# Lcrypto/mod-interleaveavx_multithreads-FAID

Measured on AMD Instinct MI355X. Metric: decoded Gb/s @ 10 iters, 50G-PON LDPC; FER match vs AVX512 ref, higher is better.
Workload: dtype i8

## Files before the change

### include/lnsfaid.h

```cpp
#ifndef LNSFAID_H
#define LNSFAID_H

#include <stddef.h>
#include <stdint.h>

#ifdef __cplusplus
extern "C" {
#endif

#define LNSFAID_GROUP 32

#define LNSFAID_OK 0
#define LNSFAID_E_INVAL (-1)
#define LNSFAID_E_CODE (-2)
#define LNSFAID_E_NOMEM (-3)
#define LNSFAID_E_HIP (-4)
#define LNSFAID_E_NODEVICE (-5)
#define LNSFAID_E_INTERNAL (-6)

typedef struct lnsfaid_code {
    int32_t n_var;
    int32_t n_check;
    int32_t n_edges;
    int32_t z;
// ... 162 lines not shown
int lnsfaid_io_buffers(lnsfaid_ctx* ctx, int8_t** d_fixInput, int8_t** d_decodedBits, lnsfaid_group_stats** d_stats);

int lnsfaid_host_register(void* ptr, size_t bytes);
int lnsfaid_host_unregister(void* ptr);

int lnsfaid_read_stats(lnsfaid_ctx* ctx, lnsfaid_group_stats* stats, size_t n_groups);

#define LNSFAID_COMM_ID_BYTES 128
int lnsfaid_comm_unique_id(uint8_t id[LNSFAID_COMM_ID_BYTES]);
int lnsfaid_comm_init(lnsfaid_ctx* ctx, int32_t n_ranks, int32_t rank, const uint8_t id[LNSFAID_COMM_ID_BYTES]);
int lnsfaid_comm_attach(lnsfaid_ctx* ctx, void* nccl_comm);
int lnsfaid_comm_destroy(lnsfaid_ctx* ctx);
int lnsfaid_allreduce_counters(lnsfaid_ctx* ctx, uint64_t counters[4]);

int lnsfaid_select_kernel(lnsfaid_ctx* ctx, int32_t rows_per_lane);
int lnsfaid_kernel_rows_per_lane(const lnsfaid_ctx* ctx);

int lnsfaid_select_waves(lnsfaid_ctx* ctx, int32_t waves_per_codeword);
int lnsfaid_kernel_waves(const lnsfaid_ctx* ctx);

#define LNSFAID_MSG_REGISTERS 1
#define LNSFAID_MSG_HBM 2
int lnsfaid_select_message_store(lnsfaid_ctx* ctx, int32_t where);
int lnsfaid_message_store(const lnsfaid_ctx* ctx);

#define LNSFAID_ZERO_SHIFT_ON 1
#define LNSFAID_ZERO_SHIFT_OFF 2
#define LNSFAID_ZERO_SHIFT_LOOP 3
#define LNSFAID_ZERO_SHIFT_STATIC 4
int lnsfaid_select_zero_shift(lnsfaid_ctx* ctx, int32_t mode);
int lnsfaid_zero_shift_groups(const lnsfaid_ctx* ctx, int32_t* groups, int32_t n);
int lnsfaid_code_zero_shift_order(const lnsfaid_code* code, int32_t* groups, int32_t* order);

int lnsfaid_kernel_residency(lnsfaid_ctx* ctx, int32_t* workgroups_per_cu, int32_t* lds_limit);


int lnsfaid_kernel_time(lnsfaid_ctx* ctx, double* out_ms, uint64_t* out_launches, int32_t reset);

void* lnsfaid_stream(lnsfaid_ctx* ctx);

const char* lnsfaid_strerror(int err);
const char* lnsfaid_last_hip_error(void);
const char* lnsfaid_version(void);

#ifdef __cplusplus
}
#endif
#endif
```

### mod-interleaveavx_multithreads-faid_amd/csrc/lnsfaid_capi.hip

```cpp
#include <hip/hip_runtime.h>

#include <dlfcn.h>
#include <rccl/rccl.h>

#include <cstdio>
#include <cstdlib>
#include <cstring>
#include <new>
#include <vector>

#include "lnsfaid_device.h"
#include "lnsfaid_quantise.h"
#include "lnsfaid_swar.h"

extern "C" hipError_t lf_launch_decode(int method, int uniform_w, const LfKernelArgs* args, size_t lds_bytes,
                                       hipStream_t stream);
extern "C" const void* lf_decode_func(int method, int uniform_w);
extern "C" int lf_decode_threads(void);
extern "C" const void* lf_decode4_func(int method, int ef, int rm);
extern "C" int lf_decode4_threads(void);
extern "C" hipError_t lf_launch_decode4(int method, int ef, int rm, const LfKernelArgs* args, size_t lds_bytes, hipStream_t stream);
extern "C" int lf_decode4_rm_layers(void);
extern "C" const void* lf_decode4cw_func(int method, int ef, int rm);
extern "C" hipError_t lf_launch_decode4cw(int method, int ef, int rm, const LfCwArgs* args, size_t lds_bytes, hipStream_t stream);
// ... 127 lines not shown
    int fe_interleave = 1;
    int fe_exact = 0;
    int fe_prefec = 0;
    unsigned long long* d_fe_prefec_frames = nullptr;
    unsigned long long* d_fe_prefec_acc = nullptr;
    uint2* d_cap_cnt = nullptr;
    unsigned long long* d_cap_meta = nullptr;
    unsigned long long* h_cap_meta = nullptr;
    size_t cap_slots = 0;
    uint32_t* d_cap_slots = nullptr;
    lnsfaid_error_record* d_cap_records = nullptr;
    int8_t* d_cap_payload = nullptr;
    unsigned long long* d_fec_acc = nullptr;
    unsigned long long* h_fec_acc = nullptr;
    int enc_state = 0;
    uint32_t* d_enc_sup = nullptr;
    uint32_t* d_enc_off = nullptr;
    unsigned long long* d_fe_keys = nullptr;
};

static int stream_wait(lnsfaid_ctx* ctx)
{
    if (sync_blocking()) {
        HIP_TRY(hipEventRecord(ctx->ev_block, ctx->stream));
        HIP_TRY(hipEventSynchronize(ctx->ev_block));
    } else {
        HIP_TRY(hipStreamSynchronize(ctx->stream));
    }
    return LNSFAID_OK;
}

static int weight_class(int w) { return w == 3 ? 0 : (w == 6 ? 1 : (w == 11 ? 2 : 3)); }

static int build_code(const lnsfaid_code* code, LfDevCode* out)
{
    memset(out, 0, sizeof(*out));
    if (!code || !code->pos_vn || !code->deg || !code->deg_rows) return LNSFAID_E_INVAL;
    const int Z = code->z, N = code->n_var, M = code->n_check, E = code->n_edges;
    if (Z != LF_Z) return LNSFAID_E_CODE;
    if (N <= 0 || M <= 0 || N % Z || M % Z || M >= N) return LNSFAID_E_CODE;
    const int nbr = M / Z, nbc = N / Z, K = N - M;
    if (nbr > LF_MAX_BR || nbc > LF_MAX_BC) return LNSFAID_E_CODE;
    if (K % 4 || M % 4 || N % LF_T) return LNSFAID_E_CODE;
    if (code->puncture_tail < 0 || code->puncture_tail > N) return LNSFAID_E_CODE;
    std::vector<int> row_deg;
    row_deg.reserve(M);
    long e_total = 0;
    for (int k = 0; k < code->nb_degres; ++k) {
        if (code->deg_rows[k] < 0 || code->deg[k] < 2 || code->deg[k] > LF_MAX_DEG) return LNSFAID_E_CODE;
        for (int i = 0; i < code->deg_rows[k]; ++i) { row_deg.push_back(code->deg[k]); e_total += code->deg[k]; }
    }
    if ((int)row_deg.size() != M || e_total != E) return LNSFAID_E_CODE;

    size_t e = 0;
    for (int br = 0; br < nbr; ++br) {
        const int deg = row_deg[(size_t)br * Z];
        out->deg[br] = deg;
        const uint16_t* row0 = code->pos_vn + e;
        for (int j = 0; j < 64; ++j) out->sbtab[br][j] = 0u;
        for (int j = 0; j < 32; ++j) out->sbplain[br][j] = 0u;
        int prev_cb = -1;
        for (int j = 0; j < deg; ++j) {
            const int cb = row0[j] / Z, sh = row0[j] % Z;
            if (row0[j] >= N || cb <= prev_cb) return LNSFAID_E_CODE;
            prev_cb = cb;
            out->circ[br][j].sb = (uint32_t)cb * (uint32_t)Z + (uint32_t)sh;
// ... 3 lines not shown
            out->cbtab[br][j] = (uint32_t)cb * (uint32_t)Z;
            if (out->col_weight[cb] >= LF_MAX_COLW) return LNSFAID_E_CODE;
            out->colcirc[cb][out->col_weight[cb]++] = (uint32_t)br | ((uint32_t)sh << 8);
        }
        for (int i = 0; i < Z; ++i) {
            if (row_deg[(size_t)br * Z + i] != deg) return LNSFAID_E_CODE;
            for (int j = 0; j < deg; ++j) {
                const uint32_t sb = out->circ[br][j].sb;
                const int want = (int)(sb / (uint32_t)Z * (uint32_t)Z + (sb % (uint32_t)Z + (uint32_t)i) % (uint32_t)Z);
                if (code->pos_vn[e + (size_t)i * deg + j] != want) return LNSFAID_E_CODE;
            }
        }
        e += (size_t)deg * Z;
        for (int j = 0; j < 32; ++j) out->zsbplain[br][j] = 0u;
        int n = 0;
        for (int zero = 1; zero >= 0; --zero)
            for (int j = 0; j < deg; ++j)
                if ((out->s4tab[br][j] == 0u) == (zero != 0)) {
                    out->zsbplain[br][n] = out->sbplain[br][j];
                    out->zs4tab[br][n] = out->s4tab[br][j];
                    out->zcbtab[br][n] = out->cbtab[br][j];
                    ++n;
                }
        int n_zero = 0;
        while (n_zero < deg && out->zs4tab[br][n_zero] == 0u) ++n_zero;
        out->zinst[br] = lf_decode4z_inst(deg, n_zero / 4);
    }
    {
        const int nw = N / 32, pw = M / 32;
        const uint32_t hard0 = lf_lds_off_hard(N), zero = lf_lds_off_zero(N, nw, pw);
        if (lf_lds_bytes(N, nw, pw) > 0xffffu) return LNSFAID_E_CODE;
        for (int br = 0; br < LF_MAX_BR; ++br)
            for (int j = 0; j < LF_MAX_DEG; ++j)
                for (int k = 0; k < 8; ++k) {
                    uint2 e; e.x = zero | (zero << 16); e.y = 0;
                    if (br < nbr && j < out->deg[br]) {
                        const uint32_t sb = out->circ[br][j].sb, cb = sb / (uint32_t)Z, sh = sb % (uint32_t)Z;
                        const uint32_t o = (32u * (uint32_t)k + sh) & 255u, q = o >> 5;
                        e.x = (hard0 + 4u * (cb * 8u + q)) | ((hard0 + 4u * (cb * 8u + ((q + 1u) & 7u))) << 16);
                        e.y = o & 31u;
                    }
                    out->synw[br][j][k] = e;
                }
    }
    for (int br = 0; br < nbr; ++br)
        for (int j = 0; j < out->deg[br]; ++j)
            out->circ[br][j].wclass = (uint32_t)weight_class(out->col_weight[out->circ[br][j].sb / (uint32_t)Z]);
    out->n_var = N; out->n_check = M; out->k_info = K; out->nbr = nbr; out->nbc = nbc;
    out->puncture_tail = code->puncture_tail;
    out->n_words = N / 32; out->p_words = M / 32;
    return LNSFAID_OK;
}

static void build_wcols(LfDevCode* code, int W)
{
    code->n_wcols = 0;
    for (int cb = 0; cb < code->nbc; ++cb)
        if (code->col_weight[cb] == W) code->wcol[code->n_wcols++] = cb;
    bool seen[LF_MAX_BC] = {};
    for (int br = 0; br < LF_MAX_BR; ++br) {
        code->era_edges[br] = 0;
        for (int j = 0; br < code->nbr && j < code->deg[br]; ++j) {
            const int cb = (int)(code->circ[br][j].sb / LF_Z);
            if (code->col_weight[cb] == W && !seen[cb]) { seen[cb] = true; code->era_edges[br] |= 1u << j; }
        }
    }
}

static int build_cfg(const lnsfaid_cfg* cfg, LfDevCfg* out)
{
    if (!cfg) return LNSFAID_E_INVAL;
    if (cfg->decode_method < 0 || cfg->decode_method > 5) return LNSFAID_E_INVAL;
    if (cfg->max_iteration < 0 || cfg->max_iteration > (1 << 20)) return LNSFAID_E_INVAL;
    if (cfg->max_bf_iter < 0 || cfg->max_bf_iter > (1 << 20)) return LNSFAID_E_INVAL;
    if (cfg->regular_col_weight < 0 || cfg->regular_col_weight > LF_MAX_COLW) return LNSFAID_E_INVAL;
    memset(out, 0, sizeof(*out));
    out->method = cfg->decode_method;
    out->max_iter = cfg->max_iteration;
    out->factor_1 = cfg->decode_method == 0 ? (int16_t)cfg->factor_1 : (int8_t)cfg->factor_1;
    out->factor_2 = cfg->decode_method == 0 ? (int16_t)cfg->factor_2 : (int8_t)cfg->factor_2;
    out->floor_err_count = cfg->floor_err_count;
    out->floor_iter_thresh = cfg->floor_iter_thresh;
    out->ef = cfg->ef_elimination;
    out->max_bf = (cfg->decode_method == 0 || cfg->decode_method == 1) ? 0 : cfg->max_bf_iter;
    out->L0 = cfg->bf_L0; out->L1 = cfg->bf_L1; out->alpha = cfg->bf_alpha; out->delta = cfg->bf_delta;
    out->W = cfg->regular_col_weight;
    out->hard2_thr = cfg->hard2_threshold;
    out->vote_cap = (int8_t)cfg->bf_vote_cap;
    if ((cfg->decode_method == 1 || cfg->decode_method == 3 || cfg->decode_method == 4)
        && ((int8_t)cfg->factor_1 < 0 || (int8_t)cfg->factor_2 < 1)) return LNSFAID_E_INVAL;
    if (cfg->decode_method == 5 && cfg->ef_elimination != 1) return LNSFAID_E_INVAL;
    if (cfg->decode_method == 2 && (cfg->ef_elimination < 0 || cfg->ef_elimination > 2)) return LNSFAID_E_INVAL;
    if (cfg->decode_method != 2 && cfg->decode_method != 5 && cfg->ef_elimination != 0) return LNSFAID_E_INVAL;
    out->uniform_w = 1;
    for (int it = 0; it < 6; ++it)
        for (int w = 0; w < 4; ++w) {
            for (int a = 0; a < 8; ++a) {
                const int v = cfg->v2c_map[it][w][a], ve = cfg->v2c_map_ef[it][w][a];
// ... 257 lines not shown
    ctx->zero_shift = mode;
    return LNSFAID_OK;
}

extern "C" int lnsfaid_zero_shift_groups(const lnsfaid_ctx* ctx, int32_t* groups, int32_t n)
{
    if (!ctx || n < 0 || (n > 0 && !groups)) return LNSFAID_E_INVAL;
    const bool on = use_zero_shift(ctx);
    for (int br = 0; br < n; ++br) groups[br] = (on && br < ctx->hcode.nbr) ? layer_zero_groups(ctx, br) : 0;
    return on ? (use_static_layers(ctx) ? 2 : 1) : 0;
}

extern "C" int lnsfaid_code_zero_shift_order(const lnsfaid_code* code, int32_t* groups, int32_t* order)
{
    LfDevCode* dc = new (std::nothrow) LfDevCode;
    if (!dc) return LNSFAID_E_NOMEM;
    const int rc = build_code(code, dc);
    if (rc) { delete dc; return rc; }
    const int nbr = dc->nbr;
    for (int br = 0; br < nbr; ++br) {
        int n_zero = 0;
        while (n_zero < dc->deg[br] && dc->zs4tab[br][n_zero] == 0u) ++n_zero;
        if (groups) groups[br] = n_zero / 4;
        for (int j = 0; order && j < LF_MAX_DEG; ++j) {
            order[br * LF_MAX_DEG + j] = -1;
            for (int i = 0; j < dc->deg[br] && i < dc->deg[br]; ++i)
                if (dc->cbtab[br][i] == dc->zcbtab[br][j] && dc->s4tab[br][i] == dc->zs4tab[br][j]) order[br * LF_MAX_DEG + j] = i;
        }
    }
    delete dc;
    return nbr;
}

static bool cw_possible(const lnsfaid_ctx* ctx) { return ctx->waves_per_cw != 2 && use_kernel4(ctx); }

static bool packed_kernel(const lnsfaid_ctx* ctx) { return use_kernel4(ctx) && !use_kernel5(ctx); }

static const void* selected_kernel(const lnsfaid_ctx* ctx, int* threads, int rule, bool packed = false)
{
    if (packed) {
        *threads = lf_decode4_threads();
        return lf_decode4p_func(ctx->hcfg.method, ctx->hcfg.ef, use_msg_registers(ctx) ? 1 : 0, rule == LNSFAID_STOP_CODEWORD ? 1 : 0);
    }
    if (rule == LNSFAID_STOP_CODEWORD) {
        *threads = lf_decode4_threads();
        return cw_possible(ctx) ? lf_decode4cw_func(ctx->hcfg.method, ctx->hcfg.ef, use_msg_registers(ctx) ? 1 : 0) : nullptr;
    }
    if (use_kernel5(ctx)) {
        *threads = lf_decode5_threads();
        return lf_decode5_func(ctx->hcfg.method);
    }
    if (use_zero_shift(ctx)) {
        *threads = lf_decode4_threads();
        return use_static_layers(ctx) ? lf_decode4s_func(ctx->hcfg.method) : lf_decode4z_func(ctx->hcfg.method);
    }
    if (use_kernel4(ctx)) {
        *threads = lf_decode4_threads();
        return lf_decode4_func(ctx->hcfg.method, ctx->hcfg.ef, use_msg_registers(ctx) ? 1 : 0);
    }
    *threads = lf_decode_threads();
    return lf_decode_func(ctx->hcfg.method, ctx->hcfg.uniform_w);
}

extern "C" int lnsfaid_select_message_store(lnsfaid_ctx* ctx, int32_t where)
{
    if (!ctx || where < 0 || where > LNSFAID_MSG_HBM) return LNSFAID_E_INVAL;
// ... 1562 lines not shown
```

### mod-interleaveavx_multithreads-faid_amd/csrc/lnsfaid_device.h

```cpp
#ifndef LNSFAID_DEVICE_H
#define LNSFAID_DEVICE_H

#include <stdint.h>

#include "lnsfaid.h"

#define LF_Z 256
#define LF_T 128
#define LF_MAX_BR 32
#define LF_MAX_DEG 24
#define LF_MAX_BC 256
#define LF_MAX_COLW 16

#define LF_DONE 0x40000000
#define LF_PROG_MASK 0x0fffffff

#define LF_JCODE_A(j) ((j) < 16 ? (j) : (j) + 16)
#define LF_JCODE_B(j) ((j) < 16 ? (j) + 16 : (j) + 32)

struct LfCirc {
    uint32_t sb;
    uint32_t wclass;
};

struct LfDevCode {
    int32_t n_var, n_check, k_info, nbr, nbc, puncture_tail, n_words , p_words ;
    int32_t n_wcols;
    int32_t deg[LF_MAX_BR];
    LfCirc circ[LF_MAX_BR][LF_MAX_DEG];
    uint32_t sbtab[LF_MAX_BR][64];
    uint32_t sbplain[LF_MAX_BR][32];
    uint32_t s4tab[LF_MAX_BR][LF_MAX_DEG];
    uint32_t cbtab[LF_MAX_BR][LF_MAX_DEG];
    uint2 synw[LF_MAX_BR][LF_MAX_DEG][8];
    int32_t col_weight[LF_MAX_BC];
    int32_t wcol[LF_MAX_BC];
    uint32_t era_edges[LF_MAX_BR];
    uint32_t colcirc[LF_MAX_BC][LF_MAX_COLW];
    uint32_t zsbplain[LF_MAX_BR][32];
    uint32_t zs4tab[LF_MAX_BR][LF_MAX_DEG];
    uint32_t zcbtab[LF_MAX_BR][LF_MAX_DEG];
    int32_t zinst[LF_MAX_BR];
};

struct LfDevCfg {
    int32_t method, max_iter, factor_1, factor_2, floor_err_count, floor_iter_thresh, ef, max_bf;
    int32_t L0, L1, alpha, delta, W, hard2_thr, vote_cap;
    int32_t uniform_w;
    int32_t bf_fast;
    int32_t nms_fits;
    uint32_t nms_t[4];
    uint32_t lut_lo[6][4], lut_hi[6][4];
    uint32_t lut_ef_lo[6][4], lut_ef_hi[6][4];
};

struct LfLaneState {
    int32_t Th, l0, l1, t;
};

struct LfKernelArgs {
    const LfDevCode* code;
    const LfDevCfg* cfg;
    const int8_t* fix_input;
    int8_t* decoded;
    int8_t* st_en;
    uint4* st_rows;
    uint32_t* st_bits;
    LfLaneState* st_lane;
    const int32_t* status_cur;
    int32_t* status_next;
    uint32_t* remaining;
    int32_t* live;
    lnsfaid_group_stats* stats;
    int32_t n_cw;
};
// ... 31 lines not shown
```

### mod-interleaveavx_multithreads-faid_amd/csrc/lnsfaid_phases.h

```cpp
#ifndef LNSFAID_PHASES_H
#define LNSFAID_PHASES_H

#ifndef LF_WG_SYNC
#define LF_WG_SYNC() __syncthreads()
#endif

#include <hip/hip_runtime.h>

#include "lnsfaid_device.h"

typedef const __attribute__((address_space(4))) LfDevCode* CCode;
typedef const __attribute__((address_space(4))) LfDevCfg* CCfg;

__device__ __forceinline__ int imin(int a, int b) { return a < b ? a : b; }
__device__ __forceinline__ int imax(int a, int b) { return a > b ? a : b; }

template <int T>
__device__ __forceinline__ int block_sum(int wave_value, int tid, int* sRed)
{
    if (T == 64) {
        LF_WG_SYNC();
        return wave_value;
    }
    if ((tid & 63) == 0) sRed[tid >> 6] = wave_value;
    LF_WG_SYNC();
    int total = 0;
    for (int w = 0; w < T / 64; ++w) total += sRed[w];
    LF_WG_SYNC();
    return total;
}

__device__ __forceinline__ void window64(const uint32_t* blk, uint32_t o, uint32_t& lo, uint32_t& hi)
{
    const uint32_t q = o >> 5, r = o & 31u;
    const uint32_t w0 = blk[q & 7u], w1 = blk[(q + 1u) & 7u], w2 = blk[(q + 2u) & 7u];
    lo = __builtin_amdgcn_alignbit(w1, w0, r);
    hi = __builtin_amdgcn_alignbit(w2, w1, r);
}

__device__ __forceinline__ int add_reduce32(int v)
{
    v += __builtin_amdgcn_update_dpp(0, v, 0x111, 0xf, 0xf, false);
    v += __builtin_amdgcn_update_dpp(0, v, 0x112, 0xf, 0xf, false);
    v += __builtin_amdgcn_update_dpp(0, v, 0x114, 0xf, 0xf, false);
    v += __builtin_amdgcn_update_dpp(0, v, 0x118, 0xf, 0xf, false);
    v += __builtin_amdgcn_update_dpp(0, v, 0x142, 0xa, 0xf, false);
    return v;
}

#define LF_SYN_ROUNDS 3
#define LF_SYN_JP (LF_MAX_DEG / 2)
struct SynCache {
    uint2 e[LF_SYN_ROUNDS][LF_SYN_JP];
};
__device__ __forceinline__ bool syn_cache_fits(int nbr) { return nbr * 16 <= LF_SYN_ROUNDS * 64; }
__device__ __forceinline__ void syn_cache_load(const LfDevCode* gc, int nbr, int tid, SynCache& sc)
{
#pragma unroll
    for (int r = 0; r < LF_SYN_ROUNDS; ++r) {
        const int ht = tid + 64 * r;
        const int task = ht < nbr * 16 ? ht >> 1 : 0, part = ht & 1;
#pragma unroll
        for (int j = 0; j < LF_SYN_JP; ++j) sc.e[r][j] = gc->synw[task >> 3][part * LF_SYN_JP + j][task & 7];
    }
}

template <int T, bool ROWBITS, bool CACHED = false>
__device__ __forceinline__ int syndrome(CCode c, const LfDevCode* gc, uint32_t* sP, int tid, uint32_t& pA, uint32_t& pB, int* sRed,
                        const SynCache* sc = nullptr)
{
    typedef const __attribute__((address_space(3))) uint32_t lds_u32;
    const int nbr = c->nbr;
    int cnt = 0;
    if (CACHED) {
        static_assert(!CACHED || T == 64, "register tables: one-wave kernel only");
#pragma unroll
        for (int r = 0; r < LF_SYN_ROUNDS; ++r) {
            const int ht = tid + 64 * r;
            if (ht < nbr * 16) {
                uint32_t acc = 0;
                uint32_t w0[LF_SYN_JP], w1[LF_SYN_JP];
#pragma unroll
                for (int j = 0; j < LF_SYN_JP; ++j) {
                    const uint2 e = sc->e[r][j];
                    w0[j] = *(lds_u32*)(size_t)(e.x & 0xffffu); w1[j] = *(lds_u32*)(size_t)(e.x >> 16);
                }
                __builtin_amdgcn_sched_barrier(0);
#pragma unroll
                for (int j = 0; j < LF_SYN_JP; ++j) acc ^= __builtin_amdgcn_alignbit(w1[j], w0[j], sc->e[r][j].y);
                acc ^= (uint32_t)__builtin_amdgcn_mov_dpp((int)acc, 0xb1, 0xf, 0xf, false);
                if (!(ht & 1)) {
                    sP[ht >> 1] = acc;
                    cnt += __popc(acc);
                }
            }
        }
    } else
// ... 24 lines not shown
        uint32_t a = 0, b = 0;
        const uint32_t* p = sP + (tid >> 5);
        const uint32_t sh = (uint32_t)tid & 31u;
        for (int br = 0; br < nbr; ++br) {
            a |= ((p[br * 8] >> sh) & 1u) << br;
            b |= ((p[br * 8 + 4] >> sh) & 1u) << br;
        }
        pA = a; pB = b;
    }
    return total;
}

__device__ __forceinline__ int bit_of(const uint32_t* words, int v) { return (int)((words[v >> 5] >> (v & 31)) & 1u); }

#define LF_BF_ROUNDS 4
struct BfCache {
    uint32_t cc[LF_BF_ROUNDS][3];
    int w0[LF_BF_ROUNDS];
};
__device__ __forceinline__ bool bf_cache_fits(CCode c, CCfg f) { return f->bf_fast && c->n_wcols * 4 <= LF_BF_ROUNDS * 64; }
__device__ __forceinline__ void bf_cache_load(CCode c, const LfDevCode* gc, int tid, BfCache& bc)
{
    const int units = c->n_wcols * 4;
#pragma unroll
    for (int r = 0; r < LF_BF_ROUNDS; ++r) {
        const int u = tid + 64 * r;
        const int cb = gc->wcol[u < units ? u >> 2 : 0];
        bc.w0[r] = cb * 8 + 2 * (u & 3);
#pragma unroll
        for (int k = 0; k < 3; ++k) bc.cc[r][k] = gc->colcirc[cb][k];
    }
}

template <int T, int METHOD, bool CACHED = false>
__device__ __forceinline__ void bf_step(CCode c, CCfg f, const LfDevCode* gc, uint32_t* sHard, const uint32_t* sHard0, uint32_t* sHard2,
                        const uint32_t* sP, int tid, LfLaneState& ls, int* sRed, const BfCache* bc = nullptr)
{
    const int W = f->W;
    int Th = ls.Th, l0 = ls.l0, l1 = ls.l1;
    if (!ls.t) Th = imax(Th - f->delta, -128);
    const bool max_Th = ls.t && (l0 < (int)(int8_t)f->L0);
    if (max_Th) { Th = (int8_t)(W + f->alpha); l0 = imin(l0 + 1, 127); }
    const bool submax_Th = ls.t && !max_Th && (l1 < (int)(int8_t)f->L1);
    if (submax_Th) { Th = (int8_t)(W + f->alpha - f->delta); l1 = imin(l1 + 1, 127); }
    if (ls.t && !max_Th && !submax_Th) Th = (int8_t)(W + f->alpha - 2 * f->delta);
    Th = imax(Th, 1);
    const bool big = Th >= (int)(int8_t)W;
    const int alpha = (int8_t)f->alpha;
    int any = 0;

    if (f->bf_fast) {
        const int units = c->n_wcols * 4;
        static_assert(!CACHED || T == 64, "register tables: one-wave kernel only");
        auto unit = [&](int u, uint32_t cc0, uint32_t cc1, uint32_t cc2, int w0) {
            const uint32_t win = (uint32_t)(u & 3);
            const uint32_t cc[3] = { cc0, cc1, cc2 };
            uint32_t plo[3], phi[3];
#pragma unroll
            for (int k = 0; k < 3; ++k)
                window64(sP + (cc[k] & 0xffu) * 8u, (64u * win - ((cc[k] >> 8) & 0xffu)) & 255u, plo[k], phi[k]);
#pragma unroll
            for (int h = 0; h < 2; ++h) {
                const uint32_t p1 = h ? phi[0] : plo[0], p2 = h ? phi[1] : plo[1], p3 = h ? phi[2] : plo[2];
                const uint32_t hd = sHard[w0 + h];
                const uint32_t fl = alpha ? (hd ^ sHard0[w0 + h]) : 0u;
                const uint32_t s0 = p1 ^ p2 ^ p3, cy = (p1 & p2) | (p1 & p3) | (p2 & p3);
                uint32_t m;
                if (Th <= 1) m = s0 | cy | fl;
                else if (Th == 2) m = cy | (s0 & fl);
                else if (Th == 3) m = cy & (s0 | fl);
                else if (Th == 4) m = cy & s0 & fl;
                else m = 0u;
                any |= (m != 0u);
                if (METHOD == 5) {
                    const uint32_t h2 = sHard2[w0 + h];
                    if (big) { sHard[w0 + h] = hd ^ m; sHard2[w0 + h] = h2 ^ m; }
                    else { sHard[w0 + h] = hd ^ (m & ~h2); sHard2[w0 + h] = h2 & ~m; }
                } else {
                    sHard[w0 + h] = hd ^ m;
// ... 20 lines not shown
                const int x = tid + half * T;
                const int v = cb * LF_Z + x;
                int vote = 0;
                for (int k = 0; k < W; ++k) {
                    const uint32_t cc = gc->colcirc[cb][k];
                    vote += bit_of(sP, (int)((cc & 0xffu) << 8) + (int)(((uint32_t)x - ((cc >> 8) & 0xffu)) & 0xffu));
                }
                const int flipped = bit_of(sHard, v) ^ bit_of(sHard0, v);
                const int fl = (imin(vote + (flipped ? alpha : 0), 127) >= Th) ? 1 : 0;
                const unsigned long long fm = __ballot(fl);
                any |= (fm != 0ull);
                if ((tid & 63) == 0) {
                    const int w = v >> 5;
#pragma unroll
                    for (int h = 0; h < 2; ++h) {
                        const uint32_t m = (uint32_t)(fm >> (32 * h));
                        if (METHOD == 5) {
                            const uint32_t h2 = sHard2[w + h];
                            if (big) { sHard[w + h] ^= m; sHard2[w + h] = h2 ^ m; }
                            else { sHard[w + h] ^= m & ~h2; sHard2[w + h] = h2 & ~m; }
                        } else {
                            sHard[w + h] ^= m;
                        }
                    }
                }
            }
        }
    }
    ls.Th = Th; ls.l0 = l0; ls.l1 = l1;
    const unsigned long long anyw = __ballot(any);
    ls.t = block_sum<T>(anyw != 0ull ? 1 : 0, tid, sRed) != 0;
}

__device__ __forceinline__ uint32_t votes_ge(uint32_t c3, uint32_t c2, uint32_t c1, uint32_t c0, int k)
{
    uint32_t lt = 0u, eqm = 0xffffffffu;
    const uint32_t pl[4] = { c0, c1, c2, c3 };
#pragma unroll
    for (int b = 3; b >= 0; --b) {
        if ((k >> b) & 1) { lt |= eqm & ~pl[b]; eqm &= pl[b]; }
        else eqm &= ~pl[b];
    }
    return ~lt;
}

template <int T>
__device__ __forceinline__ void bf_step_plain(CCode c, CCfg f, const LfDevCode* gc, uint32_t* sHard, uint32_t* sCnt, const uint32_t* sP, int tid,
                              int* sRed)
{
    const int nw = c->n_words;
    const int units = c->nbc * 4;
    uint32_t seen = 0;
    for (int u = tid; u < units; u += T) {
        const int cb = u >> 2;
        const uint32_t win = (uint32_t)(u & 3);
        const int wgt = gc->col_weight[cb];
        uint32_t c0[2] = { 0u, 0u }, c1[2] = { 0u, 0u }, c2[2] = { 0u, 0u }, c3[2] = { 0u, 0u };
        for (int k = 0; k < wgt; ++k) {
            const uint32_t cc = gc->colcirc[cb][k];
            uint32_t x[2];
            window64(sP + (cc & 0xffu) * 8u, (64u * win - ((cc >> 8) & 0xffu)) & 255u, x[0], x[1]);
#pragma unroll
            for (int h = 0; h < 2; ++h) {
                uint32_t carry = x[h], t;
                t = c0[h] & carry; c0[h] ^= carry; carry = t;
                t = c1[h] & carry; c1[h] ^= carry; carry = t;
// ... 37 lines not shown
```

### mod-interleaveavx_multithreads-faid_amd/csrc/lnsfaid_rows4.h

```cpp
#ifndef LNSFAID_ROWS4_H
#define LNSFAID_ROWS4_H

#include "lnsfaid_device.h"
#include "lnsfaid_phases.h"
#include "lnsfaid_swar.h"

#define LF_T4 64

#define LF4_OMS(M) ((M) == 1 || (M) == 3 || (M) == 4)

struct DevTab4 {
    CCode c;
    int br;
    uint32_t sbv;
    __device__ __forceinline__ uint32_t sb(int j) const { return c->circ[br][j].sb; }
    __device__ __forceinline__ uint32_t s4(int j) const { return c->s4tab[br][j]; }
    __device__ __forceinline__ uint32_t cb256(int j) const { return c->cbtab[br][j]; }
    __device__ __forceinline__ uint32_t sb_dyn4(uint32_t idx4) const
    {
        return (uint32_t)__builtin_amdgcn_ds_bpermute((int)idx4, (int)sbv);
    }
};

typedef __attribute__((address_space(3))) uint32_t lds4_u32;
// ... 383 lines not shown
                                                                                      \
                build_erasure_plane4(c, a.code, sHard, sP, f->W, tid_i);                                                                                                                                 \
                LF4_MAIN_STEP<METHOD, EF2, RM>(c, f, a.code, g_rows, R, tid_i, prog, sP, true, lme, lf_lds_off_hard(N));                                                                                 \
            } else {                                                                                                                                                                                     \
                LF4_MAIN_STEP<METHOD, false, RM>(c, f, a.code, g_rows, R, tid_i, prog, sP, have_par && needs_checksums, lme, 0u);                                                                        \
            }                                                                                                                                                                                            \
            prog++;                                                                                                                                                                                      \
        }                                                                                                                                                                                                \

#define LF4_ENTER_BF() \
        if (!parked && prog < t_end) {                                                                                          \
                                      \
            uint32_t conf[LF_MAX_BC * 8 / LF_T4];                           \
            if (METHOD == 5) {                                                                                                  \
                build_plane4<true>(c, sHard, f->hard2_thr, tid);                       \
_Pragma("unroll")                                                                                                               \
                for (int k = 0; k < LF_MAX_BC * 8 / LF_T4; ++k) conf[k] = (tid + k * LF_T4 < nw) ? sHard[tid + k * LF_T4] : 0u; \
                LF_WG_SYNC();                                                                                                   \
            }                                                                                                                   \
            build_plane4<false>(c, sHard, 0, tid);                                                                              \
                                                        \
            copy_out<9>(sHard0, sHard, nw, tid);                                                                                \
            if (METHOD == 5) {                                                                                                  \
_Pragma("unroll")                                                                                                               \
                for (int k = 0; k < LF_MAX_BC * 8 / LF_T4; ++k) if (tid + k * LF_T4 < nw) sHard2[tid + k * LF_T4] = conf[k];    \
            }                                                                                                                   \
            ls.Th = (int8_t)f->W; ls.l0 = 0; ls.l1 = 0; ls.t = 1;                                                               \
            in_bf = true;                                                                                                       \
            LF_WG_SYNC();                                                                                                       \
        }                                                                                                                       \

#define LF4_BF_LOOPS() \
    if (in_bf && !parked) {                                                                                                                 \
        if ((RM || syn_cache_fits(c->nbr)) && (METHOD == 3 || bf_cache_fits(c, f))) {                                                       \
            SynCache sc;                                                                                                                    \
            BfCache bc;                                                                                                                     \
            syn_cache_load(a.code, c->nbr, tid, sc);                                                                                        \
            if (METHOD != 3) bf_cache_load(c, a.code, tid, bc);                                                                             \
            while (prog < t_end) {                                                                                                          \
                const int unsat = syndrome<LF_T4, false, true>(c, a.code, sP, tid, pA, pB, sRed, &sc);                                      \
                if (unsat == 0 && LF4_CLEAN_STOPS(tid)) { parked = true; break; }                                                           \
                LF4_ON_PASS(tid)                                                                                                            \
                if (METHOD == 3) bf_step_plain<LF_T4>(c, f, a.code, sHard, sHard2 + nw , sP, tid, sRed); \
                else bf_step<LF_T4, METHOD, true>(c, f, a.code, sHard, sHard0, sHard2, sP, tid, ls, sRed, &bc);                             \
                prog++;                                                                                                                     \
            }                                                                                                                               \
        } else {                                                                                                                            \
            while (prog < t_end) {                                                                                                          \
                const int unsat = syndrome<LF_T4, false>(c, a.code, sP, tid, pA, pB, sRed);                                                 \
                if (unsat == 0 && LF4_CLEAN_STOPS(tid)) { parked = true; break; }                                                           \
                LF4_ON_PASS(tid)                                                                                                            \
                if (METHOD == 3) bf_step_plain<LF_T4>(c, f, a.code, sHard, sHard2 + nw , sP, tid, sRed); \
                else bf_step<LF_T4, METHOD>(c, f, a.code, sHard, sHard0, sHard2, sP, tid, ls, sRed);                                        \
                prog++;                                                                                                                     \
            }                                                                                                                               \
        }                                                                                                                                   \
    }                                                                                                                                       \

#endif
```

### mod-interleaveavx_multithreads-faid_amd/pyabi.py

```python
import ctypes as C
import os

HERE = os.path.dirname(os.path.abspath(__file__))
LIB_PATH = os.path.join(HERE, "csrc", "liblnsfaid.so")

GROUP = 32
MSG_REGISTERS, MSG_HBM = 1, 2
ZERO_SHIFT_ON, ZERO_SHIFT_OFF, ZERO_SHIFT_LOOP, ZERO_SHIFT_STATIC = 1, 2, 3, 4
STOP_GROUP, STOP_CODEWORD = 0, 1


class Code(C.Structure):
    _fields_ = [
        ("n_var", C.c_int32),
        ("n_check", C.c_int32),
        ("n_edges", C.c_int32),
        ("z", C.c_int32),
        ("puncture_tail", C.c_int32),
        ("nb_degres", C.c_int32),
        ("deg", C.POINTER(C.c_int32)),
        ("deg_rows", C.POINTER(C.c_int32)),
        ("pos_vn", C.POINTER(C.c_uint16)),
    ]

# ... 77 lines not shown
                                          C.POINTER(C.c_uint64), C.POINTER(C.c_uint64)]),
    "lnsfaid_fec_status_packed_host": (C.c_int, [C.POINTER(Code), C.c_void_p, C.c_void_p, C.c_void_p, C.c_size_t, C.c_void_p,
                                                 C.POINTER(C.c_uint64), C.POINTER(C.c_uint64)]),
    "lnsfaid_fec_status_device": (C.c_int, [C.c_void_p, C.c_void_p, C.c_void_p, C.c_void_p, C.c_size_t, C.c_void_p,
                                            C.POINTER(C.c_uint64), C.POINTER(C.c_uint64)]),
    "lnsfaid_fec_status_packed_device": (C.c_int, [C.c_void_p, C.c_void_p, C.c_void_p, C.c_void_p, C.c_size_t, C.c_void_p,
                                                   C.POINTER(C.c_uint64), C.POINTER(C.c_uint64)]),
    "lnsfaid_frontend_set_frames": (C.c_int, [C.c_void_p, C.c_void_p, C.c_void_p, C.c_size_t]),
    "lnsfaid_frontend_input_bits": (C.c_int, [C.c_void_p, C.POINTER(C.c_void_p)]),
    "lnsfaid_code_parity_inverse": (C.c_int, [C.POINTER(Code), C.c_void_p, C.c_size_t]),
    "lnsfaid_encode_device": (C.c_int, [C.c_void_p, C.c_void_p, C.c_size_t, C.c_void_p]),
    "lnsfaid_encode": (C.c_int, [C.c_void_p, C.c_void_p, C.c_size_t, C.c_void_p]),
    "lnsfaid_frontend_random_frames": (C.c_int, [C.c_void_p, C.POINTER(C.c_uint64), C.c_size_t]),
    "lnsfaid_io_buffers": (C.c_int, [C.c_void_p, C.POINTER(C.c_void_p), C.POINTER(C.c_void_p), C.POINTER(C.c_void_p)]),
    "lnsfaid_read_stats": (C.c_int, [C.c_void_p, C.c_void_p, C.c_size_t]),
    "lnsfaid_host_register": (C.c_int, [C.c_void_p, C.c_size_t]),
    "lnsfaid_host_unregister": (C.c_int, [C.c_void_p]),
    "lnsfaid_comm_unique_id": (C.c_int, [C.c_void_p]),
    "lnsfaid_comm_init": (C.c_int, [C.c_void_p, C.c_int32, C.c_int32, C.c_void_p]),
    "lnsfaid_comm_attach": (C.c_int, [C.c_void_p, C.c_void_p]),
    "lnsfaid_comm_destroy": (C.c_int, [C.c_void_p]),
    "lnsfaid_allreduce_counters": (C.c_int, [C.c_void_p, C.POINTER(C.c_uint64)]),
    "lnsfaid_select_kernel": (C.c_int, [C.c_void_p, C.c_int32]),
    "lnsfaid_kernel_rows_per_lane": (C.c_int, [C.c_void_p]),
    "lnsfaid_select_waves": (C.c_int, [C.c_void_p, C.c_int32]),
    "lnsfaid_frontend_set_exact": (C.c_int, [C.c_void_p, C.c_int32]),
    "lnsfaid_frontend_fastpath_bounds": (C.c_int, [C.c_void_p, C.POINTER(C.c_double), C.POINTER(C.c_double)]),
    "lnsfaid_kernel_waves": (C.c_int, [C.c_void_p]),
    "lnsfaid_select_message_store": (C.c_int, [C.c_void_p, C.c_int32]),
    "lnsfaid_message_store": (C.c_int, [C.c_void_p]),
    "lnsfaid_select_zero_shift": (C.c_int, [C.c_void_p, C.c_int32]),
    "lnsfaid_zero_shift_groups": (C.c_int, [C.c_void_p, C.POINTER(C.c_int32), C.c_int32]),
    "lnsfaid_code_zero_shift_order": (C.c_int, [C.POINTER(Code), C.POINTER(C.c_int32), C.POINTER(C.c_int32)]),
    "lnsfaid_kernel_residency": (C.c_int, [C.c_void_p, C.POINTER(C.c_int32), C.POINTER(C.c_int32)]),
    "lnsfaid_kernel_time": (C.c_int, [C.c_void_p, C.POINTER(C.c_double), C.POINTER(C.c_uint64), C.c_int32]),
    "lnsfaid_stream": (C.c_void_p, [C.c_void_p]),
    "lnsfaid_strerror": (C.c_char_p, [C.c_int]),
    "lnsfaid_last_hip_error": (C.c_char_p, []),
    "lnsfaid_version": (C.c_char_p, []),
}


def bind(lib, symbols):
    for name, (res, args) in symbols.items():
        fn = getattr(lib, name)
        fn.restype = res
        fn.argtypes = args
    return lib


_lib = None


def load():
    global _lib
    if _lib is None:
        if not os.path.exists(LIB_PATH):
            raise RuntimeError(
                "HIP extension %s is missing: run `python -c 'import __graft_entry__ as g; g.build()'` "
                "(no CPU fallback exists in the product path)" % LIB_PATH)
        _lib = bind(C.CDLL(LIB_PATH), SYMBOLS)
    return _lib


class Code50GPON:

    def __init__(self, lib=None):
        lib = lib or load()
        self.pos_vn = (C.c_uint16 * 70400)()
        self.deg = (C.c_int32 * 3)()
        self.deg_rows = (C.c_int32 * 3)()
        self.code = Code()
        rc = lib.lnsfaid_code_50gpon(C.byref(self.code), self.pos_vn, self.deg, self.deg_rows)
        if rc != 0:
            raise RuntimeError("lnsfaid_code_50gpon failed: %d" % rc)

    @property
    def N(self):
        return self.code.n_var

    @property
    def M(self):
        return self.code.n_check

    @property
    def K(self):
        return self.code.n_var - self.code.n_check


def code_zero_shift_order(code, lib=None):
    lib = lib or load()
    groups, order = (C.c_int32 * 32)(), (C.c_int32 * (32 * 24))()
    nbr = lib.lnsfaid_code_zero_shift_order(C.byref(code), groups, order)
    if nbr < 0:
        raise ValueError("lnsfaid_code_zero_shift_order failed: %d" % nbr)
    return list(groups[:nbr]), [[j for j in order[br * 24:br * 24 + 24] if j >= 0] for br in range(nbr)]


def default_cfg(method, max_iter, lib=None):
    lib = lib or load()
    cfg = Cfg()
    rc = lib.lnsfaid_cfg_default(C.byref(cfg), method, max_iter)
    if rc != 0:
        raise ValueError("lnsfaid_cfg_default(%d, %d) failed: %d" % (method, max_iter, rc))
    return cfg


def pack_llr4(fix_input, lib=None):
    import numpy as np
    lib = lib or load()
    fix_input = np.ascontiguousarray(fix_input, dtype=np.int8)
    out = np.empty(fix_input.size // 2, dtype=np.uint8)
    rc = lib.lnsfaid_pack_llr4(fix_input.ctypes.data, fix_input.size, out.ctypes.data)
    if rc != 0:
        raise ValueError("lnsfaid_pack_llr4 failed: %d" % rc)
    return out


def unpack_bits(bits, lib=None):
    import numpy as np
    lib = lib or load()
    bits = np.ascontiguousarray(bits, dtype=np.uint32)
    out = np.empty(bits.size * 32, dtype=np.int8)
    rc = lib.lnsfaid_unpack_bits(bits.ctypes.data, out.size, out.ctypes.data)
    if rc != 0:
        raise ValueError("lnsfaid_unpack_bits failed: %d" % rc)
    return out


# ... 374 lines not shown
```

Before: 83.20.

## Stage BF syndrome with precomputed fixed-column base and register-resident flip addresses

Splits the per-row syndrome into a contribution from columns that bit-flipping never changes and one from the flippable weight-W columns. The fixed part is computed once into registers before the BF loop, so each BF pass only re-reads the few flippable columns. Flip-step LDS addresses, shifts and thresholds are also precomputed into a BfStage struct, and the step uses explicit LDS pointers with scheduling barriers. This adds register pressure and a fallback when more than 14 flippable edges fall in one row. A host API for inspecting the split tables is included.

New measurement: 84.40, median of 6. +1.4%, better.

```diff
diff --git a/include/lnsfaid.h b/include/lnsfaid.h
--- a/include/lnsfaid.h
+++ b/include/lnsfaid.h
@@ -218,6 +218,8 @@
 int lnsfaid_zero_shift_groups(const lnsfaid_ctx* ctx, int32_t* groups, int32_t n);
 int lnsfaid_code_zero_shift_order(const lnsfaid_code* code, int32_t* groups, int32_t* order);
 
+int lnsfaid_code_bf_walk(const lnsfaid_code* code, int32_t col_weight, uint32_t* full, uint32_t* flipped, uint32_t* fixed, int32_t* info);
+
 int lnsfaid_kernel_residency(lnsfaid_ctx* ctx, int32_t* workgroups_per_cu, int32_t* lds_limit);
 
 
diff --git a/mod-interleaveavx_multithreads-faid_amd/csrc/lnsfaid_capi.hip b/mod-interleaveavx_multithreads-faid_amd/csrc/lnsfaid_capi.hip
--- a/mod-interleaveavx_multithreads-faid_amd/csrc/lnsfaid_capi.hip
+++ b/mod-interleaveavx_multithreads-faid_amd/csrc/lnsfaid_capi.hip
@@ -183,6 +183,22 @@
 
 static int weight_class(int w) { return w == 3 ? 0 : (w == 6 ? 1 : (w == 11 ? 2 : 3)); }
 
+static uint2 syn_entry(uint32_t hard0, uint32_t sb, int k)
+{
+    const uint32_t cb = sb / (uint32_t)LF_Z, sh = sb % (uint32_t)LF_Z;
+    const uint32_t o = (32u * (uint32_t)k + sh) & 255u, q = o >> 5;
+    uint2 e;
+    e.x = (hard0 + 4u * (cb * 8u + q)) | ((hard0 + 4u * (cb * 8u + ((q + 1u) & 7u))) << 16);
+    e.y = o & 31u;
+    return e;
+}
+static uint2 syn_zero_entry(uint32_t zero)
+{
+    uint2 e;
+    e.x = zero | (zero << 16); e.y = 0;
+    return e;
+}
+
 static int build_code(const lnsfaid_code* code, LfDevCode* out)
 {
     memset(out, 0, sizeof(*out));
@@ -252,16 +268,8 @@
         if (lf_lds_bytes(N, nw, pw) > 0xffffu) return LNSFAID_E_CODE;
         for (int br = 0; br < LF_MAX_BR; ++br)
             for (int j = 0; j < LF_MAX_DEG; ++j)
-                for (int k = 0; k < 8; ++k) {
-                    uint2 e; e.x = zero | (zero << 16); e.y = 0;
-                    if (br < nbr && j < out->deg[br]) {
-                        const uint32_t sb = out->circ[br][j].sb, cb = sb / (uint32_t)Z, sh = sb % (uint32_t)Z;
-                        const uint32_t o = (32u * (uint32_t)k + sh) & 255u, q = o >> 5;
-                        e.x = (hard0 + 4u * (cb * 8u + q)) | ((hard0 + 4u * (cb * 8u + ((q + 1u) & 7u))) << 16);
-                        e.y = o & 31u;
-                    }
-                    out->synw[br][j][k] = e;
-                }
+                for (int k = 0; k < 8; ++k)
+                    out->synw[br][j][k] = (br < nbr && j < out->deg[br]) ? syn_entry(hard0, out->circ[br][j].sb, k) : syn_zero_entry(zero);
     }
     for (int br = 0; br < nbr; ++br)
         for (int j = 0; j < out->deg[br]; ++j)
@@ -284,6 +292,22 @@
             const int cb = (int)(code->circ[br][j].sb / LF_Z);
             if (code->col_weight[cb] == W && !seen[cb]) { seen[cb] = true; code->era_edges[br] |= 1u << j; }
         }
+    }
+    const uint32_t hard0 = lf_lds_off_hard(code->n_var), zero = lf_lds_off_zero(code->n_var, code->n_words, code->p_words);
+    code->bfw_fits = 1;
+    for (int br = 0; br < LF_MAX_BR; ++br) {
+        int nw = 0, nc = 0;
+        for (int j = 0; br < code->nbr && j < code->deg[br]; ++j) {
+            const uint32_t sb = code->circ[br][j].sb;
+            const bool w = code->col_weight[sb / LF_Z] == W;
+            if (w && nw == 2 * LF_BFW_JP) { code->bfw_fits = 0; continue; }
+            for (int k = 0; k < 8; ++k) (w ? code->synw_w[br][nw] : code->synw_c[br][nc])[k] = syn_entry(hard0, sb, k);
+            ++(w ? nw : nc);
+        }
+        for (; nw < 2 * LF_BFW_JP; ++nw)
+            for (int k = 0; k < 8; ++k) code->synw_w[br][nw][k] = syn_zero_entry(zero);
+        for (; nc < LF_MAX_DEG; ++nc)
+            for (int k = 0; k < 8; ++k) code->synw_c[br][nc][k] = syn_zero_entry(zero);
     }
 }
 
@@ -607,6 +631,36 @@
     return nbr;
 }
 
+extern "C" int lnsfaid_code_bf_walk(const lnsfaid_code* code, int32_t col_weight, uint32_t* full, uint32_t* flipped, uint32_t* fixed, int32_t* info)
+{
+    if (!full || !flipped || !fixed || !info || col_weight < 0 || col_weight > LF_MAX_COLW) return LNSFAID_E_INVAL;
+    LfDevCode* dc = new (std::nothrow) LfDevCode;
+    if (!dc) return LNSFAID_E_NOMEM;
+    const int rc = build_code(code, dc);
+    if (rc) { delete dc; return rc; }
+    build_wcols(dc, col_weight);
+    const int nbr = dc->nbr;
+    for (int br = 0; br < nbr; ++br)
+        for (int k = 0; k < 8; ++k) {
+            for (int j = 0; j < LF_MAX_DEG; ++j) {
+                uint32_t* o = full + ((br * LF_MAX_DEG + j) * 8 + k) * 2, *x = fixed + ((br * LF_MAX_DEG + j) * 8 + k) * 2;
+                o[0] = dc->synw[br][j][k].x; o[1] = dc->synw[br][j][k].y;
+                x[0] = dc->synw_c[br][j][k].x; x[1] = dc->synw_c[br][j][k].y;
+            }
+            for (int j = 0; j < 2 * LF_BFW_JP; ++j) {
+                uint32_t* o = flipped + ((br * 2 * LF_BFW_JP + j) * 8 + k) * 2;
+                o[0] = dc->synw_w[br][j][k].x; o[1] = dc->synw_w[br][j][k].y;
+            }
+        }
+    info[0] = (int32_t)lf_lds_off_hard(dc->n_var);
+    info[1] = (int32_t)lf_lds_off_zero(dc->n_var, dc->n_words, dc->p_words);
+    info[2] = 2 * LF_BFW_JP;
+    info[3] = dc->bfw_fits;
+    info[4] = dc->n_wcols;
+    delete dc;
+    return nbr;
+}
+
 static bool cw_possible(const lnsfaid_ctx* ctx) { return ctx->waves_per_cw != 2 && use_kernel4(ctx); }
 
 static bool packed_kernel(const lnsfaid_ctx* ctx) { return use_kernel4(ctx) && !use_kernel5(ctx); }
diff --git a/mod-interleaveavx_multithreads-faid_amd/csrc/lnsfaid_device.h b/mod-interleaveavx_multithreads-faid_amd/csrc/lnsfaid_device.h
--- a/mod-interleaveavx_multithreads-faid_amd/csrc/lnsfaid_device.h
+++ b/mod-interleaveavx_multithreads-faid_amd/csrc/lnsfaid_device.h
@@ -11,6 +11,7 @@
 #define LF_MAX_DEG 24
 #define LF_MAX_BC 256
 #define LF_MAX_COLW 16
+#define LF_BFW_JP 7
 
 #define LF_DONE 0x40000000
 #define LF_PROG_MASK 0x0fffffff
@@ -41,6 +42,9 @@
     uint32_t zs4tab[LF_MAX_BR][LF_MAX_DEG];
     uint32_t zcbtab[LF_MAX_BR][LF_MAX_DEG];
     int32_t zinst[LF_MAX_BR];
+    uint2 synw_w[LF_MAX_BR][2 * LF_BFW_JP][8];
+    uint2 synw_c[LF_MAX_BR][LF_MAX_DEG][8];
+    int32_t bfw_fits;
 };
 
 struct LfDevCfg {
diff --git a/mod-interleaveavx_multithreads-faid_amd/csrc/lnsfaid_phases.h b/mod-interleaveavx_multithreads-faid_amd/csrc/lnsfaid_phases.h
--- a/mod-interleaveavx_multithreads-faid_amd/csrc/lnsfaid_phases.h
+++ b/mod-interleaveavx_multithreads-faid_amd/csrc/lnsfaid_phases.h
@@ -54,15 +54,20 @@
     uint2 e[LF_SYN_ROUNDS][LF_SYN_JP];
 };
 __device__ __forceinline__ bool syn_cache_fits(int nbr) { return nbr * 16 <= LF_SYN_ROUNDS * 64; }
-__device__ __forceinline__ void syn_cache_load(const LfDevCode* gc, int nbr, int tid, SynCache& sc)
+template <int JP>
+__device__ __forceinline__ void syn_table_load(const uint2 (*tab)[2 * JP][8], int nbr, int tid, uint2 (&e)[LF_SYN_ROUNDS][JP])
 {
 #pragma unroll
     for (int r = 0; r < LF_SYN_ROUNDS; ++r) {
         const int ht = tid + 64 * r;
         const int task = ht < nbr * 16 ? ht >> 1 : 0, part = ht & 1;
 #pragma unroll
-        for (int j = 0; j < LF_SYN_JP; ++j) sc.e[r][j] = gc->synw[task >> 3][part * LF_SYN_JP + j][task & 7];
-    }
+        for (int j = 0; j < JP; ++j) e[r][j] = tab[task >> 3][part * JP + j][task & 7];
+    }
+}
+__device__ __forceinline__ void syn_cache_load(const LfDevCode* gc, int nbr, int tid, SynCache& sc)
+{
+    syn_table_load<LF_SYN_JP>(gc->synw, nbr, tid, sc.e);
 }
 
 template <int T, bool ROWBITS, bool CACHED = false>
@@ -153,19 +158,34 @@
     }
 }
 
+struct BfThr {
+    int W, alpha, delta, L0, L1;
+};
+__device__ __forceinline__ BfThr bf_thr_load(CCfg f)
+{
+    BfThr p;
+    p.W = f->W; p.alpha = f->alpha; p.delta = f->delta; p.L0 = f->L0; p.L1 = f->L1;
+    return p;
+}
+__device__ __forceinline__ void bf_threshold(const BfThr& p, const LfLaneState& ls, int& Th, int& l0, int& l1)
+{
+    Th = ls.Th; l0 = ls.l0; l1 = ls.l1;
+    if (!ls.t) Th = imax(Th - p.delta, -128);
+    const bool max_Th = ls.t && (l0 < (int)(int8_t)p.L0);
+    if (max_Th) { Th = (int8_t)(p.W + p.alpha); l0 = imin(l0 + 1, 127); }
+    const bool submax_Th = ls.t && !max_Th && (l1 < (int)(int8_t)p.L1);
+    if (submax_Th) { Th = (int8_t)(p.W + p.alpha - p.delta); l1 = imin(l1 + 1, 127); }
+    if (ls.t && !max_Th && !submax_Th) Th = (int8_t)(p.W + p.alpha - 2 * p.delta);
+    Th = imax(Th, 1);
+}
+
 template <int T, int METHOD, bool CACHED = false>
 __device__ __forceinline__ void bf_step(CCode c, CCfg f, const LfDevCode* gc, uint32_t* sHard, const uint32_t* sHard0, uint32_t* sHard2,
                         const uint32_t* sP, int tid, LfLaneState& ls, int* sRed, const BfCache* bc = nullptr)
 {
     const int W = f->W;
-    int Th = ls.Th, l0 = ls.l0, l1 = ls.l1;
-    if (!ls.t) Th = imax(Th - f->delta, -128);
-    const bool max_Th = ls.t && (l0 < (int)(int8_t)f->L0);
-    if (max_Th) { Th = (int8_t)(W + f->alpha); l0 = imin(l0 + 1, 127); }
-    const bool submax_Th = ls.t && !max_Th && (l1 < (int)(int8_t)f->L1);
-    if (submax_Th) { Th = (int8_t)(W + f->alpha - f->delta); l1 = imin(l1 + 1, 127); }
-    if (ls.t && !max_Th && !submax_Th) Th = (int8_t)(W + f->alpha - 2 * f->delta);
-    Th = imax(Th, 1);
+    int Th, l0, l1;
+    bf_threshold(bf_thr_load(f), ls, Th, l0, l1);
     const bool big = Th >= (int)(int8_t)W;
     const int alpha = (int8_t)f->alpha;
     int any = 0;
@@ -252,6 +272,168 @@
     ls.t = block_sum<T>(anyw != 0ull ? 1 : 0, tid, sRed) != 0;
 }
 
+typedef __attribute__((address_space(3))) uint32_t lf_lds_u32;
+struct BfStage {
+    uint2 e[LF_SYN_ROUNDS][LF_BFW_JP];
+    uint32_t base[LF_SYN_ROUNDS];
+    uint32_t wa[LF_BF_ROUNDS][3][3];
+    uint32_t wr[LF_BF_ROUNDS][3];
+    uint32_t ah[LF_BF_ROUNDS];
+    BfThr thr;
+    int half_tasks, units;
+    uint32_t h0_off, h2_off;
+    uint32_t amask;
+};
+__device__ __forceinline__ bool bf_stage_fits(CCode c, CCfg f) { return bf_cache_fits(c, f) && c->bfw_fits; }
+__device__ __forceinline__ void bf_stage_load(CCode c, CCfg f, const LfDevCode* gc, int tid, BfStage& bs)
+{
+    const int nbr = c->nbr;
+    const uint32_t hard0 = lf_lds_off_hard(c->n_var), par0 = lf_lds_off_p(c->n_var, c->n_words);
+    bs.thr = bf_thr_load(f);
+    bs.half_tasks = nbr * 16; bs.units = c->n_wcols * 4;
+    bs.h0_off = 0u - hard0; bs.h2_off = 4u * (uint32_t)c->n_words - hard0;
+    bs.amask = (int8_t)bs.thr.alpha ? 0xffffffffu : 0u;
+    {
+        uint2 ec[LF_SYN_ROUNDS][LF_SYN_JP];
+        syn_table_load<LF_SYN_JP>(gc->synw_c, nbr, tid, ec);
+#pragma unroll
+        for (int r = 0; r < LF_SYN_ROUNDS; ++r) {
+            uint32_t w0[LF_SYN_JP], w1[LF_SYN_JP], acc = 0;
+#pragma unroll
+            for (int j = 0; j < LF_SYN_JP; ++j) {
+                w0[j] = *(const lf_lds_u32*)(size_t)(ec[r][j].x & 0xffffu); w1[j] = *(const lf_lds_u32*)(size_t)(ec[r][j].x >> 16);
+            }
+            __builtin_amdgcn_sched_barrier(0);
+#pragma unroll
+            for (int j = 0; j < LF_SYN_JP; ++j) acc ^= __builtin_amdgcn_alignbit(w1[j], w0[j], ec[r][j].y);
+            bs.base[r] = acc;
+        }
+    }
+    syn_table_load<LF_BFW_JP>(gc->synw_w, nbr, tid, bs.e);
+    const int units = bs.units;
+#pragma unroll
+    for (int r = 0; r < LF_BF_ROUNDS; ++r) {
+        const int u = tid + 64 * r;
+        const int cb = gc->wcol[u < units ? u >> 2 : 0];
+        const uint32_t win = (uint32_t)(u & 3);
+        bs.ah[r] = hard0 + 4u * ((uint32_t)cb * 8u + 2u * win);
+#pragma unroll
+        for (int k = 0; k < 3; ++k) {
+            const uint32_t cc = gc->colcirc[cb][k];
+            const uint32_t o = (64u * win - ((cc >> 8) & 0xffu)) & 255u, q = o >> 5;
+            bs.wr[r][k] = o & 31u;
+#pragma unroll
+            for (uint32_t i = 0; i < 3; ++i) bs.wa[r][k][i] = par0 + 4u * ((cc & 0xffu) * 8u + ((q + i) & 7u));
+        }
+    }
+}
+
+__device__ __forceinline__ int syndrome_staged(uint32_t* sP, int tid, int* sRed, const BfStage& bs)
+{
+    uint32_t w0[LF_SYN_ROUNDS][LF_BFW_JP], w1[LF_SYN_ROUNDS][LF_BFW_JP];
+#pragma unroll
+    for (int r = 0; r < LF_SYN_ROUNDS; ++r)
+#pragma unroll
+        for (int j = 0; j < LF_BFW_JP; ++j) {
+            w0[r][j] = *(const lf_lds_u32*)(size_t)(bs.e[r][j].x & 0xffffu); w1[r][j] = *(const lf_lds_u32*)(size_t)(bs.e[r][j].x >> 16);
+        }
+    __builtin_amdgcn_sched_barrier(0);
+    int cnt = 0;
+#pragma unroll
+    for (int r = 0; r < LF_SYN_ROUNDS; ++r) {
+        const int ht = tid + 64 * r;
+        uint32_t acc = bs.base[r];
+#pragma unroll
+        for (int j = 0; j < LF_BFW_JP; ++j) acc ^= __builtin_amdgcn_alignbit(w1[r][j], w0[r][j], bs.e[r][j].y);
+        acc ^= (uint32_t)__builtin_amdgcn_mov_dpp((int)acc, 0xb1, 0xf, 0xf, false);
+        if (!(ht & 1) && ht < bs.half_tasks) {
+            sP[ht >> 1] = acc;
+            cnt += __popc(acc);
+        }
+    }
+    cnt = add_reduce32(cnt);
+    const int wave_cnt = __builtin_amdgcn_readlane(cnt, 31) + __builtin_amdgcn_readlane(cnt, 63);
+    return block_sum<64>(wave_cnt, tid, sRed);
+}
+
+template <int TH>
+__device__ __forceinline__ void bf_masks_staged(uint32_t (&m)[LF_BF_ROUNDS][2], const uint32_t (&s0)[LF_BF_ROUNDS][2],
+                                                const uint32_t (&cy)[LF_BF_ROUNDS][2], const uint32_t (&fl)[LF_BF_ROUNDS][2])
+{
+#pragma unroll
+    for (int r = 0; r < LF_BF_ROUNDS; ++r)
+#pragma unroll
+        for (int h = 0; h < 2; ++h)
+            m[r][h] = TH == 1 ? (s0[r][h] | cy[r][h] | fl[r][h]) : TH == 2 ? (cy[r][h] | (s0[r][h] & fl[r][h]))
+                    : TH == 3 ? (cy[r][h] & (s0[r][h] | fl[r][h])) : (cy[r][h] & s0[r][h] & fl[r][h]);
+}
+
+template <int METHOD>
+__device__ __forceinline__ void bf_step_staged(int tid, LfLaneState& ls, int* sRed, const BfStage& bs)
+{
+    int Th, l0, l1;
+    bf_threshold(bs.thr, ls, Th, l0, l1);
+    const int units = bs.units;
+    const uint32_t h2_off = bs.h2_off, amask = bs.amask;
+    uint32_t pw[LF_BF_ROUNDS][3][3], hd[LF_BF_ROUNDS][2], h0[LF_BF_ROUNDS][2], h2[LF_BF_ROUNDS][2];
+#pragma unroll
+    for (int r = 0; r < LF_BF_ROUNDS; ++r) {
+#pragma unroll
+        for (int k = 0; k < 3; ++k)
+#pragma unroll
+            for (int i = 0; i < 3; ++i) pw[r][k][i] = *(const lf_lds_u32*)(size_t)bs.wa[r][k][i];
+        const lf_lds_u32* ph = (const lf_lds_u32*)(size_t)bs.ah[r];
+        const lf_lds_u32* p0 = (const lf_lds_u32*)(size_t)(bs.ah[r] + bs.h0_off);
+        const lf_lds_u32* p2 = (const lf_lds_u32*)(size_t)(bs.ah[r] + h2_off);
+#pragma unroll
+        for (int h = 0; h < 2; ++h) {
+            hd[r][h] = ph[h]; h0[r][h] = p0[h];
+            h2[r][h] = METHOD == 5 ? p2[h] : 0u;
+        }
+    }
+    __builtin_amdgcn_sched_barrier(0);
+    uint32_t s0[LF_BF_ROUNDS][2], cy[LF_BF_ROUNDS][2], fl[LF_BF_ROUNDS][2], m[LF_BF_ROUNDS][2];
+#pragma unroll
+    for (int r = 0; r < LF_BF_ROUNDS; ++r)
+#pragma unroll
+        for (int h = 0; h < 2; ++h) {
+            uint32_t p[3];
+#pragma unroll
+            for (int k = 0; k < 3; ++k) p[k] = __builtin_amdgcn_alignbit(pw[r][k][h + 1], pw[r][k][h], bs.wr[r][k]);
+            s0[r][h] = p[0] ^ p[1] ^ p[2]; cy[r][h] = (p[0] & p[1]) | (p[0] & p[2]) | (p[1] & p[2]);
+            fl[r][h] = (hd[r][h] ^ h0[r][h]) & amask;
+        }
+    if (Th <= 1) bf_masks_staged<1>(m, s0, cy, fl);
+    else if (Th == 2) bf_masks_staged<2>(m, s0, cy, fl);
+    else if (Th == 3) bf_masks_staged<3>(m, s0, cy, fl);
+    else if (Th == 4) bf_masks_staged<4>(m, s0, cy, fl);
+    else {
+#pragma unroll
+        for (int r = 0; r < LF_BF_ROUNDS; ++r) m[r][0] = m[r][1] = 0u;
+    }
+    const bool big = Th >= 3;
+    uint32_t anym = 0;
+#pragma unroll
+    for (int r = 0; r < LF_BF_ROUNDS; ++r)
+        if (tid + 64 * r < units) {
+            anym |= m[r][0] | m[r][1];
+            lf_lds_u32* ph = (lf_lds_u32*)(size_t)bs.ah[r];
+            if (METHOD == 5) {
+                lf_lds_u32* p2 = (lf_lds_u32*)(size_t)(bs.ah[r] + h2_off);
+#pragma unroll
+                for (int h = 0; h < 2; ++h) {
+                    ph[h] = hd[r][h] ^ (big ? m[r][h] : m[r][h] & ~h2[r][h]);
+                    p2[h] = big ? h2[r][h] ^ m[r][h] : h2[r][h] & ~m[r][h];
+                }
+            } else {
+                ph[0] = hd[r][0] ^ m[r][0]; ph[1] = hd[r][1] ^ m[r][1];
+            }
+        }
+    ls.Th = Th; ls.l0 = l0; ls.l1 = l1;
+    const unsigned long long anyw = __ballot(anym != 0u);
+    ls.t = block_sum<64>(anyw != 0ull ? 1 : 0, tid, sRed) != 0;
+}
+
 __device__ __forceinline__ uint32_t votes_ge(uint32_t c3, uint32_t c2, uint32_t c1, uint32_t c0, int k)
 {
     uint32_t lt = 0u, eqm = 0xffffffffu;
diff --git a/mod-interleaveavx_multithreads-faid_amd/csrc/lnsfaid_rows4.h b/mod-interleaveavx_multithreads-faid_amd/csrc/lnsfaid_rows4.h
--- a/mod-interleaveavx_multithreads-faid_amd/csrc/lnsfaid_rows4.h
+++ b/mod-interleaveavx_multithreads-faid_amd/csrc/lnsfaid_rows4.h
@@ -439,17 +439,26 @@
 
 #define LF4_BF_LOOPS() \
     if (in_bf && !parked) {                                                                                                                 \
-        if ((RM || syn_cache_fits(c->nbr)) && (METHOD == 3 || bf_cache_fits(c, f))) {                                                       \
+        if (METHOD != 3 && (RM || syn_cache_fits(c->nbr)) && bf_stage_fits(c, f)) {                                                         \
+                                                                \
+            BfStage bs;                                                                                                                     \
+            bf_stage_load(c, f, a.code, tid, bs);                                                                                           \
+            while (prog < t_end) {                                                                                                          \
+                const int unsat = syndrome_staged(sP, tid, sRed, bs);                                                                       \
+                if (unsat == 0 && LF4_CLEAN_STOPS(tid)) { parked = true; break; }                                                           \
+                LF4_ON_PASS(tid)                                                                                                            \
+                bf_step_staged<METHOD>(tid, ls, sRed, bs);                                                                                  \
+                prog++;                                                                                                                     \
+            }                                                                                                                               \
+        } else if (METHOD == 3 && (RM || syn_cache_fits(c->nbr))) {                                                                         \
+                                                 \
             SynCache sc;                                                                                                                    \
-            BfCache bc;                                                                                                                     \
             syn_cache_load(a.code, c->nbr, tid, sc);                                                                                        \
-            if (METHOD != 3) bf_cache_load(c, a.code, tid, bc);                                                                             \
             while (prog < t_end) {                                                                                                          \
                 const int unsat = syndrome<LF_T4, false, true>(c, a.code, sP, tid, pA, pB, sRed, &sc);                                      \
                 if (unsat == 0 && LF4_CLEAN_STOPS(tid)) { parked = true; break; }                                                           \
                 LF4_ON_PASS(tid)                                                                                                            \
-                if (METHOD == 3) bf_step_plain<LF_T4>(c, f, a.code, sHard, sHard2 + nw , sP, tid, sRed); \
-                else bf_step<LF_T4, METHOD, true>(c, f, a.code, sHard, sHard0, sHard2, sP, tid, ls, sRed, &bc);                             \
+                bf_step_plain<LF_T4>(c, f, a.code, sHard, sHard2 + nw , sP, tid, sRed);                  \
                 prog++;                                                                                                                     \
             }                                                                                                                               \
         } else {                                                                                                                            \
diff --git a/mod-interleaveavx_multithreads-faid_amd/pyabi.py b/mod-interleaveavx_multithreads-faid_amd/pyabi.py
--- a/mod-interleaveavx_multithreads-faid_amd/pyabi.py
+++ b/mod-interleaveavx_multithreads-faid_amd/pyabi.py
@@ -133,6 +133,8 @@
     "lnsfaid_select_zero_shift": (C.c_int, [C.c_void_p, C.c_int32]),
     "lnsfaid_zero_shift_groups": (C.c_int, [C.c_void_p, C.POINTER(C.c_int32), C.c_int32]),
     "lnsfaid_code_zero_shift_order": (C.c_int, [C.POINTER(Code), C.POINTER(C.c_int32), C.POINTER(C.c_int32)]),
+    "lnsfaid_code_bf_walk": (C.c_int, [C.POINTER(Code), C.c_int32, C.POINTER(C.c_uint32), C.POINTER(C.c_uint32), C.POINTER(C.c_uint32),
+                                      C.POINTER(C.c_int32)]),
     "lnsfaid_kernel_residency": (C.c_int, [C.c_void_p, C.POINTER(C.c_int32), C.POINTER(C.c_int32)]),
     "lnsfaid_kernel_time": (C.c_int, [C.c_void_p, C.POINTER(C.c_double), C.POINTER(C.c_uint64), C.c_int32]),
     "lnsfaid_stream": (C.c_void_p, [C.c_void_p]),
@@ -196,6 +198,20 @@
     if nbr < 0:
         raise ValueError("lnsfaid_code_zero_shift_order failed: %d" % nbr)
     return list(groups[:nbr]), [[j for j in order[br * 24:br * 24 + 24] if j >= 0] for br in range(nbr)]
+
+
+def code_bf_walk(code, col_weight, lib=None):
+    import numpy as np
+    lib = lib or load()
+    full, fixed = np.zeros((32, 24, 8, 2), np.uint32), np.zeros((32, 24, 8, 2), np.uint32)
+    flipped = np.zeros((32 * 24 * 8 * 2,), np.uint32)
+    info = (C.c_int32 * 5)()
+    u32 = lambda x: x.ctypes.data_as(C.POINTER(C.c_uint32))
+    nbr = lib.lnsfaid_code_bf_walk(C.byref(code), col_weight, u32(full), u32(flipped), u32(fixed), info)
+    if nbr < 0:
+        raise ValueError("lnsfaid_code_bf_walk failed: %d" % nbr)
+    slots = info[2]
+    return full[:nbr], flipped[:nbr * slots * 16].reshape(nbr, slots, 8, 2), fixed[:nbr], tuple(info)
 
 
 def default_cfg(method, max_iter, lib=None):
```
